# vbronetskyi/nclt-slam-project

Hardware: AMD Instinct MI355X
Metric: relocalization frames/sec @640x480, 10k-landmark DB; Hamming-match HBM GB/s (higher is better)
Workload: dtype u8; 1 GPU; 640x480 BGR frames, 10000-record landmark DB (640000 descriptors, rows=fixed64), global relocalization tick per frame: ORB(500) + whole-DB mutual Hamming scan + top-25 PnP-RANSAC(200); frames resident in HBM, every frame's 96-byte result record written to pinned host memory by the tick's last kernel; distinct_frames=32, preroll_steps=20, streams=4, records=10000, descriptors=640000, parallelism=frames sharded across ranks, database replicated, no collective

## Files before the change

nclt-slam-project_amd/csrc/reloc_ctx.hip:

```cpp
#include <stdarg.h>
#include <stdlib.h>

#include "reloc_internal.h"

static thread_local char g_err[512] = "";

void reloc_set_error(const char *fmt, ...)
{
    va_list ap;
    va_start(ap, fmt);
    vsnprintf(g_err, sizeof(g_err), fmt, ap);
    va_end(ap);
}

RELOC_API const char *reloc_last_error(void) { return g_err; }

RELOC_API int reloc_device_count(void)
{
    int n = 0;
    if (hipGetDeviceCount(&n) != hipSuccess) return 0;
    return n;
}

template <typename T>
static int dalloc(T **p, int64_t count)
{
    HIP_TRY(hipMalloc((void **)p, (size_t)(count > 0 ? count : 1) * sizeof(T)));
    return 0;
}

static int ctx_alloc(reloc_ctx *c)
{
    int rc = 0;
    const int64_t mf = c->max_feat;
    int64_t pyr = 0;
    for (int l = 0; l < NLEV; ++l) {
        double s = pow(RELOC_ORB_SCALE_FACTOR, (double)l);
        int64_t w = (int64_t)(c->max_w / s) + 2, h = (int64_t)(c->max_h / s) + 2;
        pyr += ((w + 63) / 64 * 64) * h + 256;
    }
    c->pyr_bytes = pyr;
    rc |= dalloc(&c->pyr, pyr);
    rc |= dalloc(&c->blur, pyr);
    rc |= dalloc(&c->nms, pyr);
    rc |= dalloc(&c->rz_tab, (int64_t)NLEV * 2 * 2 * (c->max_w > c->max_h ? c->max_w : c->max_h));
    rc |= dalloc((char **)&c->pyr_tiles, (int64_t)((c->max_w + 15) / 16) * ((c->max_h + 15) / 16) * 128);
    rc |= dalloc(&c->hist, NLEV * 256);
    rc |= dalloc(&c->cand_cnt, NLEV);
    rc |= dalloc(&c->cand_key, (int64_t)NLEV * RELOC_ORB_STAGE1_CAP);
    rc |= dalloc(&c->cand_resp, (int64_t)NLEV * RELOC_ORB_STAGE1_CAP);
    rc |= dalloc(&c->kp_cnt, NLEV);
    rc |= dalloc(&c->kp_key, (int64_t)NLEV * RELOC_ORB_STAGE1_CAP);
    rc |= dalloc(&c->kp_resp, (int64_t)NLEV * RELOC_ORB_STAGE1_CAP);
    rc |= dalloc(&c->f_xy, mf * 2);
    rc |= dalloc(&c->f_size, mf);
    rc |= dalloc(&c->f_angle, mf);
    rc |= dalloc(&c->f_resp, mf);
    rc |= dalloc(&c->f_oct, mf);
    rc |= dalloc(&c->f_desc, mf * 32);
    rc |= dalloc(&c->f_count, 1);
    rc |= dalloc(&c->frame_img, (int64_t)c->max_w * c->max_h * 3);
    rc |= dalloc((char **)&c->orb_const, 1024);
    rc |= dalloc(&c->dbg_cut, NLEV);
    rc |= dalloc(&c->cand_ids, MAX_CAND);
    rc |= dalloc(&c->cand_n, 1);
    rc |= dalloc(&c->m_qidx, (int64_t)MAX_CAND * MAX_REC_ROWS);
    rc |= dalloc(&c->m_tidx, (int64_t)MAX_CAND * MAX_REC_ROWS);
    rc |= dalloc(&c->m_dist, (int64_t)MAX_CAND * MAX_REC_ROWS);
    rc |= dalloc(&c->m_n, MAX_CAND);
    rc |= dalloc(&c->p_obj, (int64_t)MAX_CAND * MAX_REC_ROWS * 3);
    rc |= dalloc(&c->p_img, (int64_t)MAX_CAND * MAX_REC_ROWS * 2);
    rc |= dalloc(&c->p_Rt, (int64_t)MAX_CAND * MAX_HYP * 12);
    rc |= dalloc(&c->p_cnt, (int64_t)MAX_CAND * MAX_HYP);
    rc |= dalloc(&c->p_inl, (int64_t)MAX_CAND * MAX_REC_ROWS);
    rc |= dalloc(&c->p_out, MAX_CAND);
    rc |= dalloc(&c->tick_res, 1);
    if (hipHostMalloc((void **)&c->tick_res_host, sizeof(TickResult), hipHostMallocDefault) != hipSuccess) {
        reloc_set_error("hipHostMalloc(result record) failed");
        c->tick_res_host = nullptr;
// ... 301 lines not shown
```

nclt-slam-project_amd/csrc/reloc_internal.h:

```cpp
#pragma once
#include <hip/hip_runtime.h>
#include <stdint.h>
#include <stdio.h>
#include <string.h>

#include "../../include/reloc.h"
#include "../../include/reloc_spec.h"

#define RELOC_API extern "C" __attribute__((visibility("default")))
#define RELOC_PROF_RING 256

void reloc_set_error(const char *fmt, ...);

#define HIP_TRY(expr)                                                                      \
    do {                                                                                   \
        hipError_t e_ = (expr);                                                            \
        if (e_ != hipSuccess) {                                                            \
            reloc_set_error("%s failed: %s (%s:%d)", #expr, hipGetErrorString(e_), __FILE__, \
                            __LINE__);                                                     \
            return RELOC_E_HIP;                                                            \
        }                                                                                  \
    } while (0)

#define ARG_CHECK(cond, msg)                                 \
// ... 9 lines not shown
        if (!(c) || !(cond)) {                                \
            reloc_set_error("bad argument: %s", msg);         \
            return RELOC_E_ARG;                               \
        }                                                     \
        (void)hipSetDevice((c)->device);                      \
    } while (0)

constexpr int NLEV = RELOC_ORB_NLEVELS;
constexpr int MAX_REC_ROWS = 4096;
constexpr int MAX_CAND = 32;
constexpr int MAX_HYP = 1024;
constexpr int64_t MAX_DB_RECORDS = 0xFFFFF;

#ifndef RELOC_SCAN_NUM_VGPR
#define RELOC_SCAN_NUM_VGPR 104
#endif
#if RELOC_SCAN_NUM_VGPR > 0
#define RELOC_SCAN_VGPR_ATTR __attribute__((amdgpu_num_vgpr(RELOC_SCAN_NUM_VGPR / 2)))
#else
#define RELOC_SCAN_VGPR_ATTR
#endif
#ifndef RELOC_SMALL_PRIO
#define RELOC_SMALL_PRIO 3
#endif
#define RELOC_SMALL_KERNEL_PRIO() __builtin_amdgcn_s_setprio(RELOC_SMALL_PRIO)

struct OrbLevel {
    int w, h;
    int stride;
    int64_t off;
    float scale;
    int quota;
};

struct TickResult {
    double anchor_pose[7];
    double reproj;
    int32_t n_inl;
    int32_t lm_idx;
    int32_t outcome;
    int32_t n_candidates;
    int32_t n_features;
    int32_t relocating;
    int32_t pad[2];
};
static_assert(sizeof(TickResult) == 96, "TickResult is the 96-byte record documented in include/reloc.h");

struct AccumResult {
    double nearest_m;
    int32_t appended;
    int32_t n_kpts;
};

struct DbShare { int refs = 1; };

struct DbArena {
    DbShare *share = nullptr;
    int64_t cap_records = 0, cap_rows = 0;
    int64_t records = 0, rows = 0;
    int max_rows = 0;
    uint8_t *desc = nullptr;
    float *pts3d = nullptr;
    float *kp2d = nullptr;
    int64_t *off = nullptr;
    double *pose = nullptr;
    double *xy_heading = nullptr;
// ... 253 lines not shown
```

nclt-slam-project_amd/csrc/reloc_match.hip:

```cpp
#include <stdlib.h>
#include <new>
#include <type_traits>
#include <utility>

#include "reloc_internal.h"

typedef uint32_t u32;

__device__ __forceinline__ u32 bcnt_acc(u32 x, u32 acc)
{
    u32 r;
    asm("v_bcnt_u32_b32 %0, %1, %2" : "=v"(r) : "v"(x), "v"(acc));
    return r;
}
__device__ __forceinline__ u32 min_u16(u32 a, u32 b)
{
    u32 r;
    asm("v_min_u16 %0, %1, %2" : "=v"(r) : "v"(a), "v"(b));
    return r;
}
template <u32 IDX>
__device__ __forceinline__ u32 key_fma(u32 d, u32 c128)
{
    u32 r;
// ... 643 lines not shown
            }
#pragma unroll
    for (int j = 0; j < 4; ++j) hs[j] = add_lshl6(acc[j][0], acc[j][1]);
}

__device__ __forceinline__ void sq_load4(const uint4 *__restrict__ cur, int q0, int C, u32 (&qw)[4][8])
{
    const char *base = (const char *)cur;
#pragma unroll
    for (int jj = 0; jj < 4; ++jj) {
        const u32 o = (u32)min(q0 + jj, C - 1) << 5;
        const uint4 qa = *(const uint4 *)(base + o), qb = *(const uint4 *)(base + o + 16);
        qw[jj][0] = qa.x; qw[jj][1] = qa.y; qw[jj][2] = qa.z; qw[jj][3] = qa.w;
        qw[jj][4] = qb.x; qw[jj][5] = qb.y; qw[jj][6] = qb.z; qw[jj][7] = qb.w;
    }
}

#define SQ_N4(a, b)  "v_min_u16_dpp " a ", " a ", " a " row_shl:4 row_mask:0xf bank_mask:0x5\n\t" \
                     "v_min_u16_dpp " a ", " b ", " b " row_shr:4 row_mask:0xf bank_mask:0xa\n\t"
#define SQ_N8(a, b)  "v_min_u16_dpp " a ", " a ", " a " row_ror:8 row_mask:0xf bank_mask:0x3\n\t" \
                     "v_min_u16_dpp " a ", " b ", " b " row_ror:8 row_mask:0xf bank_mask:0xc\n\t"
#define SQ_Q1(a)     "v_min_u16_dpp " a ", " a ", " a " quad_perm:[1,0,3,2] row_mask:0xf bank_mask:0xf\n\t"
#define SQ_Q2(a)     "v_min_u16_dpp " a ", " a ", " a " quad_perm:[2,3,0,1] row_mask:0xf bank_mask:0xf\n\t"
#define SQ_NOP       "s_nop 1\n\t"
template <int G>
__device__ __forceinline__ u32 sq_bfly(u32 (&d)[G])
{
    if constexpr (G == 16) {
        asm volatile(SQ_NOP
                     SQ_N4("%0", "%1") SQ_N4("%2", "%3") SQ_N4("%4", "%5") SQ_N4("%6", "%7")
                     SQ_N4("%8", "%9") SQ_N4("%10", "%11") SQ_N4("%12", "%13") SQ_N4("%14", "%15")
                     SQ_N8("%0", "%2") SQ_N8("%4", "%6") SQ_N8("%8", "%10") SQ_N8("%12", "%14")
                     "v_permlane16_swap_b32 %0, %4\n\t"
                     "v_permlane16_swap_b32 %8, %12\n\t"
                     "v_min_u16 %0, %0, %4\n\t"
                     "v_min_u16 %8, %8, %12\n\t"
                     SQ_NOP
                     "v_permlane32_swap_b32 %0, %8\n\t"
                     "v_min_u16 %0, %0, %8\n\t"
                     SQ_NOP SQ_Q1("%0") SQ_NOP SQ_Q2("%0")
                     : "+v"(d[0]), "+v"(d[1]), "+v"(d[2]), "+v"(d[3]), "+v"(d[4]), "+v"(d[5]), "+v"(d[6]), "+v"(d[7]), "+v"(d[8]),
                       "+v"(d[9]), "+v"(d[10]), "+v"(d[11]), "+v"(d[12]), "+v"(d[13]), "+v"(d[14]), "+v"(d[15]));
    } else if constexpr (G == 8) {
        asm volatile(SQ_NOP
                     SQ_N4("%0", "%1") SQ_N4("%2", "%3") SQ_N4("%4", "%5") SQ_N4("%6", "%7")
                     SQ_N8("%0", "%2") SQ_N8("%4", "%6")
                     SQ_NOP
                     "v_permlane16_swap_b32 %0, %4\n\t"
                     "v_min_u16 %0, %0, %4\n\t"
                     SQ_NOP SQ_Q1("%0") SQ_NOP SQ_Q2("%0")
                     "v_mov_b32 %4, %0\n\t"
                     SQ_NOP
                     "v_permlane32_swap_b32 %0, %4\n\t"
                     "v_min_u16 %0, %0, %4\n\t"
                     : "+v"(d[0]), "+v"(d[1]), "+v"(d[2]), "+v"(d[3]), "+v"(d[4]), "+v"(d[5]), "+v"(d[6]), "+v"(d[7]));
    } else {
        static_assert(G == 4, "groups of 4, 8 or 16 queries");
        asm volatile(SQ_NOP
                     SQ_N4("%0", "%1") SQ_N4("%2", "%3")
                     SQ_NOP
                     SQ_N8("%0", "%2")
                     SQ_NOP SQ_Q1("%0") SQ_NOP SQ_Q2("%0")
                     "v_mov_b32 %2, %0\n\t"
                     SQ_NOP
                     "v_permlane16_swap_b32 %0, %2\n\t"
                     "v_min_u16 %0, %0, %2\n\t"
// ... 884 lines not shown
```

nclt-slam-project_amd/csrc/reloc_orb.hip:

```cpp
#include <math.h>

#include "../../include/reloc_orb_pattern.h"
#include "reloc_internal.h"

typedef uint32_t u32;

constexpr int HARRIS_CHUNK = 1024;
static_assert(HARRIS_CHUNK == 1024, "k_harris reads one dword per thread");

struct OrbTable {
    OrbLevel lev[NLEV];
    int fast_tile_base[NLEV + 1];
    int blur_tile_base[NLEV + 1];
    int flat_base[NLEV + 1];
    int rz_off[NLEV][4];
};

__constant__ signed char c_pattern[RELOC_ORB_NTESTS * 4];
__constant__ int c_umax[16] = {15, 15, 15, 15, 14, 14, 14, 13, 13, 12, 11, 10, 9, 8, 6, 3};
__constant__ signed char c_ring_dx[16] = {0, 1, 2, 3, 3, 3, 2, 1, 0, -1, -2, -3, -3, -3, -2, -1};
__constant__ signed char c_ring_dy[16] = {3, 3, 2, 1, 0, -1, -2, -3, -3, -3, -2, -1, 0, 1, 2, 3};

__device__ __forceinline__ int find_level(const int *base, int id)
{
// ... 13 lines not shown
    return p;
}

__device__ __forceinline__ int gray_fixed(int b, int g, int r, int flags)
{
    const bool c15 = flags & RELOC_GRAY_FLAG_15BIT;
    const int cb = c15 ? RELOC_GRAY15_CB : RELOC_GRAY_CB, cg = c15 ? RELOC_GRAY15_CG : RELOC_GRAY_CG, cr = c15 ? RELOC_GRAY15_CR : RELOC_GRAY_CR;
    const int sh = c15 ? RELOC_GRAY15_SHIFT : RELOC_GRAY_SHIFT;
    return (b * cb + g * cg + r * cr + (1 << (sh - 1))) >> sh;
}
static inline int gray_flags(const reloc_ctx *ctx, int order)
{
    return (order & 1) | (ctx->prm.gray_coeff_bits == RELOC_GRAY15_SHIFT ? RELOC_GRAY_FLAG_15BIT : 0);
}
__global__ __launch_bounds__(256) void k_gray_plain(const uint8_t *__restrict__ src, int w, int h, int sstride, int order_rgb,
                                                    uint8_t *__restrict__ dst)
{
    const int x = blockIdx.x * 256 + threadIdx.x, y = blockIdx.y;
    if (x >= w) return;
    const uint8_t *s = src + (size_t)y * sstride + 3 * x;
    const int c0 = s[0], c1 = s[1], c2 = s[2];
    const int b = (order_rgb & 1) ? c2 : c0, r = (order_rgb & 1) ? c0 : c2;
    dst[(size_t)y * w + x] = (uint8_t)gray_fixed(b, c1, r, order_rgb);
}

#ifndef PYR_TW
#define PYR_TW 64
#define PYR_TH 32
#endif
constexpr int PT_W = PYR_TW, PT_H = PYR_TH;
struct PyrTile {
    uint16_t o[NLEV][4];
    uint16_t n[NLEV][4];
};
static_assert(sizeof(PyrTile) == 128, "PyrTile is read as 8 dwordx4");

struct PyrLds { int lev[NLEV]; int tabs; };

struct OrbFrame {
    const OrbTable *tab; const PyrTile *tiles; const int32_t *rz; const uint8_t *src;
    uint8_t *pyr, *nms, *blur; int32_t *hist, *cand_cnt; u32 *cand_key; float *cand_resp; int32_t *dbg_cut;
    int32_t *kp_cnt; u32 *kp_key; float *kp_resp; float *f_xy, *f_size, *f_angle, *f_resp; int32_t *f_oct; uint8_t *f_desc;
    int32_t *f_count;
};
struct OrbBatch { OrbFrame f[RELOC_BATCH_MAX]; };

template <int CH, bool ALIGNED>
__device__ __forceinline__ void pyr_fetch(const uint8_t *sp, int x4, int w, u32 (&d)[3])
{
    if (ALIGNED) {
        const u32 *s4 = reinterpret_cast<const u32 *>(sp);
        d[0] = s4[0];
        if (CH == 3) { d[1] = s4[1]; d[2] = s4[2]; }
    } else {
        d[0] = d[1] = d[2] = 0;
#pragma unroll
        for (int k = 0; k < 4 * CH; ++k)
            if (x4 + k / CH < w) d[k >> 2] |= (u32)sp[k] << (8 * (k & 3));
    }
}

template <int CH>
__device__ __forceinline__ u32 pyr_gray4(const u32 (&d)[3], int x4, int w, int order_rgb)
{
    if (CH == 1) return d[0];
    u32 out = 0;
#pragma unroll
    for (int k = 0; k < 4; ++k) {
        int c[3];
#pragma unroll
        for (int j = 0; j < 3; ++j) { const int bi = 3 * k + j; c[j] = (d[bi >> 2] >> (8 * (bi & 3))) & 0xFF; }
        const int b = (order_rgb & 1) ? c[2] : c[0], r = (order_rgb & 1) ? c[0] : c[2];
        const int g = gray_fixed(b, c[1], r, order_rgb);
        if (x4 + k < w) out |= (u32)g << (8 * k);
    }
    return out;
}

__device__ __forceinline__ void pyr_tab_index(const OrbTable *__restrict__ tab, const PyrTile &T, const int (&tbase)[NLEV + 1], int i,
                                              int &po, int &pc)
{
    int j = i, nw = 0, x0 = 0, y0 = 0, ox = 0, cx = 0, oy = 0, cy = 0;
#pragma unroll
    for (int k = 1; k < NLEV; ++k) {
        const bool m = i >= tbase[k];
        j = m ? i - tbase[k] : j;
        nw = m ? T.n[k][1] - T.n[k][0] : nw;
        x0 = m ? (int)T.n[k][0] : x0;
        y0 = m ? (int)T.n[k][2] : y0;
        ox = m ? tab->rz_off[k][0] : ox;
        cx = m ? tab->rz_off[k][1] : cx;
        oy = m ? tab->rz_off[k][2] : oy;
        cy = m ? tab->rz_off[k][3] : cy;
    }
    const bool isx = j < nw;
    const int p = isx ? x0 + j : y0 + j - nw;
    po = (isx ? ox : oy) + p;
    pc = (isx ? cx : cy) + p;
}

__device__ __forceinline__ int pyr_div(int q, float inv) { return (int)(((float)q + 0.5f) * inv); }

template <int CH, bool ALIGNED, int PYR_BS>
__device__ __forceinline__ void pyramid_body(const OrbTable *__restrict__ tab, const PyrTile *__restrict__ tiles,
                                                 const int32_t *__restrict__ rz, const uint8_t *__restrict__ src, int w, int h,
                                                 int sstride, int order_rgb, uint8_t *__restrict__ pyr, PyrLds lds,
                                                 int32_t *__restrict__ hist, int32_t *__restrict__ cand_cnt)
{
    extern __shared__ u32 s_pyr[];
    const int tid = threadIdx.x;
    if (blockIdx.x == 0) {
        for (int i = tid; i < NLEV * 256; i += PYR_BS) hist[i] = 0;
        if (tid < NLEV) cand_cnt[tid] = 0;
    }
    const PyrTile &T = tiles[blockIdx.x];
    uint8_t *const base = reinterpret_cast<uint8_t *>(s_pyr);
    u32 *const tabs = s_pyr + (lds.tabs >> 2);
    int tbase[NLEV + 1];
    tbase[1] = 0;
#pragma unroll
    for (int l = 1; l < NLEV; ++l) tbase[l + 1] = tbase[l] + (T.n[l][1] - T.n[l][0]) + (T.n[l][3] - T.n[l][2]);
    constexpr int TAB_IT = 1024 / PYR_BS, L0_IT = 1536 / PYR_BS;
    u32 tv[TAB_IT][2];
#pragma unroll
    for (int it = 0; it < TAB_IT; ++it) {
        const int i = tid + it * PYR_BS;
        tv[it][0] = tv[it][1] = 0;
        if (i < tbase[NLEV]) {
            int po, pc;
            pyr_tab_index(tab, T, tbase, i, po, pc);
            tv[it][0] = (u32)rz[po];
            tv[it][1] = (u32)rz[pc];
        }
    }
    const int x00 = T.n[0][0], y00 = T.n[0][2], qpr0 = (T.n[0][1] - x00 + 3) >> 2, nq0 = qpr0 * (T.n[0][3] - y00);
    const float inv0 = 1.0f / (float)(qpr0 > 0 ? qpr0 : 1);
    u32 fv[L0_IT][3];
#pragma unroll
    for (int it = 0; it < L0_IT; ++it) {
        const int q = tid + it * PYR_BS;
        if (q < nq0) {
            const int ry = pyr_div(q, inv0), x4 = x00 + (q - ry * qpr0) * 4;
            pyr_fetch<CH, ALIGNED>(src + (size_t)(y00 + ry) * sstride + CH * x4, x4, w, fv[it]);
        }
    }
#pragma unroll
    for (int it = 0; it < TAB_IT; ++it) {
        const int i = tid + it * PYR_BS;
        if (i < tbase[NLEV]) tabs[i] = tv[it][0] | tv[it][1] << 16;
    }
#pragma unroll
    for (int it = 0; it < L0_IT; ++it) {
        const int q = tid + it * PYR_BS;
        if (q < nq0) {
            const int ry = pyr_div(q, inv0), x4 = x00 + (q - ry * qpr0) * 4;
            reinterpret_cast<u32 *>(base + lds.lev[0])[q] = pyr_gray4<CH>(fv[it], x4, w, order_rgb);
        }
    }
    for (int q = tid + L0_IT * PYR_BS; q < nq0; q += PYR_BS) {
        const int ry = pyr_div(q, inv0), x4 = x00 + (q - ry * qpr0) * 4;
        u32 d[3];
        pyr_fetch<CH, ALIGNED>(src + (size_t)(y00 + ry) * sstride + CH * x4, x4, w, d);
        reinterpret_cast<u32 *>(base + lds.lev[0])[q] = pyr_gray4<CH>(d, x4, w, order_rgb);
    }
    for (int i = tid + TAB_IT * PYR_BS; i < tbase[NLEV]; i += PYR_BS) {
        int po, pc;
        pyr_tab_index(tab, T, tbase, i, po, pc);
        tabs[i] = (u32)rz[po] | (u32)rz[pc] << 16;
    }
    __syncthreads();
#pragma unroll
    for (int l = 0; l + 1 < NLEV; ++l) {
        const int sw = tab->lev[l].w, sh = tab->lev[l].h;
        const uint8_t *cur = base + lds.lev[l];
        u32 *nxt = reinterpret_cast<u32 *>(base + lds.lev[l + 1]);
        const int nx0 = T.n[l][0], ny0 = T.n[l][2], pitch = ((T.n[l][1] - nx0 + 3) >> 2) << 2;
        const int dx0 = T.n[l + 1][0], dx1 = T.n[l + 1][1], dh = T.n[l + 1][3] - T.n[l + 1][2];
        const int qpr = (dx1 - dx0 + 3) >> 2;
        const u32 *xt = tabs + tbase[l + 1], *yt = xt + (dx1 - dx0);
        const u32 one = 1u << RELOC_RESIZE_COEF_BITS;
        const float inv = 1.0f / (float)(qpr > 0 ? qpr : 1);
        for (int q = tid; q < qpr * dh; q += PYR_BS) {
            const int ry = pyr_div(q, inv), rx4 = (q - ry * qpr) * 4;
            const u32 ye = yt[ry];
            const int sy0 = (int)(ye & 0xFFFF), sy1 = sy0 + 1 < sh ? sy0 + 1 : sh - 1;
            const u32 b = ye >> 16;
            const uint8_t *r0 = cur + (sy0 - ny0) * pitch - nx0, *r1 = cur + (sy1 - ny0) * pitch - nx0;
            u32 out = 0;
#pragma unroll
            for (int k = 0; k < 4; ++k) {
                if (dx0 + rx4 + k < dx1) {
                    const u32 xe = xt[rx4 + k];
                    const int k0 = (int)(xe & 0xFFFF), k1 = k0 + 1 < sw ? k0 + 1 : sw - 1;
                    const u32 a = xe >> 16;
                    const u32 h0 = (u32)r0[k0] * (one - a) + (u32)r0[k1] * a;
                    const u32 h1 = (u32)r1[k0] * (one - a) + (u32)r1[k1] * a;
                    const u32 v = h0 * (one - b) + h1 * b;
                    out |= ((v + (1u << 15)) >> 16) << (8 * k);
                }
            }
            nxt[q] = out;
        }
        __syncthreads();
    }
#pragma unroll
    for (int l = 0; l < NLEV; ++l) {
        const OrbLevel L = tab->lev[l];
        const uint8_t *cur = base + lds.lev[l];
        const int nx0 = T.n[l][0], ny0 = T.n[l][2], pitch = ((T.n[l][1] - nx0 + 3) >> 2) << 2;
        const int x0 = T.o[l][0], x1 = T.o[l][1], y0 = T.o[l][2], oh = T.o[l][3] - y0;
        const int qpr = (x1 - x0) >> 2;
        uint8_t *dst = pyr + L.off;
        const float inv = 1.0f / (float)(qpr > 0 ? qpr : 1);
        for (int q = tid; q < qpr * oh; q += PYR_BS) {
            const int ry = pyr_div(q, inv), x4 = x0 + (q - ry * qpr) * 4;
            u32 v = 0;
            if (x4 < L.w) {
                v = *reinterpret_cast<const u32 *>(cur + (y0 + ry - ny0) * pitch + (x4 - nx0));
                if (x4 + 4 > L.w) v &= 0xFFFFFFFFu >> (8 * (x4 + 4 - L.w));
            }
            *reinterpret_cast<u32 *>(dst + (size_t)(y0 + ry) * L.stride + x4) = v;
        }
    }
}
template <int CH, bool ALIGNED, int PYR_BS>
__global__ __launch_bounds__(PYR_BS) void k_pyramid(const OrbTable *__restrict__ tab, const PyrTile *__restrict__ tiles,
                                                 const int32_t *__restrict__ rz, const uint8_t *__restrict__ src, int w, int h,
                                                 int sstride, int order_rgb, uint8_t *__restrict__ pyr, PyrLds lds,
                                                 int32_t *__restrict__ hist, int32_t *__restrict__ cand_cnt)
{
    RELOC_SMALL_KERNEL_PRIO();
    pyramid_body<CH, ALIGNED, PYR_BS>(tab, tiles, rz, src, w, h, sstride, order_rgb, pyr, lds, hist, cand_cnt);
}
template <int CH, bool ALIGNED, int PYR_BS>
__global__ __launch_bounds__(PYR_BS) void k_pyramid_batch(OrbBatch b, int w, int h, int sstride, int order_rgb, PyrLds lds)
{
    RELOC_SMALL_KERNEL_PRIO();
    const OrbFrame &F = b.f[blockIdx.y];
    pyramid_body<CH, ALIGNED, PYR_BS>(F.tab, F.tiles, F.rz, F.src, w, h, sstride, order_rgb, F.pyr, lds, F.hist, F.cand_cnt);
}


template <bool REFLECT>
__device__ __forceinline__ u32 halo_dword(const uint8_t *__restrict__ row, int gx, int w)
{
    if (gx >= 0 && gx + 4 <= w) return *reinterpret_cast<const u32 *>(row + gx);
    u32 v = 0;
#pragma unroll
    for (int k = 0; k < 4; ++k) {
        const int x = REFLECT ? reflect101(gx + k, w) : min(max(gx + k, 0), w - 1);
        v |= (u32)row[x] << (8 * k);
    }
    return v;
}
// ... 726 lines not shown
    OrbTable tab;
    memset(&tab, 0, sizeof(tab));
    int64_t off = 0;
    for (int l = 0; l < NLEV; ++l) {
        const float s = (float)pow(RELOC_ORB_SCALE_FACTOR, (double)l);
        OrbLevel &L = tab.lev[l];
        L.scale = s;
        L.w = (int)lrintf((float)w / s);
        L.h = (int)lrintf((float)h / s);
        L.stride = (L.w + 63) / 64 * 64;
        L.off = off;
        off += ((int64_t)L.stride * L.h + 255) / 256 * 256;
    }
    if (off > ctx->pyr_bytes) { reloc_set_error("pyramid arena too small"); return RELOC_E_CAPACITY; }
    {
        const float factor = (float)(1.0 / RELOC_ORB_SCALE_FACTOR);
        float nper = (float)(nfeatures * (1 - factor) / (1 - (float)pow((double)factor, (double)NLEV)));
        int sum = 0;
        for (int l = 0; l < NLEV - 1; ++l) {
            tab.lev[l].quota = (int)lrintf(nper);
            sum += tab.lev[l].quota;
            nper *= factor;
        }
        tab.lev[NLEV - 1].quota = nfeatures - sum > 0 ? nfeatures - sum : 0;
    }
    for (int l = 0; l < NLEV; ++l) {
        const OrbLevel &L = tab.lev[l];
        tab.fast_tile_base[l + 1] = tab.fast_tile_base[l] + (L.stride / FT) * ((L.h + FT - 1) / FT);
        tab.blur_tile_base[l + 1] = tab.blur_tile_base[l] + ((L.w + BT_W - 1) / BT_W) * ((L.h + BT_H - 1) / BT_H);
        tab.flat_base[l + 1] = tab.flat_base[l] + (int)(((int64_t)L.stride * L.h + HARRIS_CHUNK - 1) / HARRIS_CHUNK);
    }
    const int maxdim = ctx->max_w > ctx->max_h ? ctx->max_w : ctx->max_h;
    int32_t *host = (int32_t *)malloc(sizeof(int32_t) * (size_t)NLEV * 4 * maxdim);
    int pos = 0;
    for (int l = 1; l < NLEV; ++l) {
        const OrbLevel &S = tab.lev[l - 1], &D = tab.lev[l];
        tab.rz_off[l][0] = pos; tab.rz_off[l][1] = pos + D.w;
        resize_axis(S.w, D.w, host + pos, host + pos + D.w);
        pos += 2 * D.w;
        tab.rz_off[l][2] = pos; tab.rz_off[l][3] = pos + D.h;
        resize_axis(S.h, D.h, host + pos, host + pos + D.h);
        pos += 2 * D.h;
    }
    const int ntx = (w + PT_W - 1) / PT_W, nty = (h + PT_H - 1) / PT_H;
    PyrTile *tiles = (PyrTile *)calloc((size_t)ntx * nty, sizeof(PyrTile));
    int lds_lev[NLEV] = {}, lds_t = 0;
    for (int t = 0; t < ntx * nty; ++t) {
        const int tx = t % ntx, ty = t / ntx;
        PyrTile &T = tiles[t];
        int nx0 = 0, nx1 = 0, ny0 = 0, ny1 = 0;
        int tsum = 0;
        for (int l = NLEV - 1; l >= 0; --l) {
            const OrbLevel &L = tab.lev[l];
            const int quads = (l == 0 ? (L.w + 3) / 4 : L.stride / 4);
            const int ox0 = 4 * (int)((int64_t)tx * quads / ntx), ox1 = 4 * (int)((int64_t)(tx + 1) * quads / ntx);
            const int oy0 = (int)((int64_t)ty * L.h / nty), oy1 = (int)((int64_t)(ty + 1) * L.h / nty);
            T.o[l][0] = (uint16_t)ox0; T.o[l][1] = (uint16_t)ox1; T.o[l][2] = (uint16_t)oy0; T.o[l][3] = (uint16_t)oy1;
            int cx0 = ox0, cx1 = ox1 < L.w ? ox1 : L.w, cy0 = oy0, cy1 = oy1;
            const bool stores = ox0 < ox1 && oy0 < oy1;
            const bool own = cx0 < cx1 && cy0 < cy1, need = nx0 < nx1 && ny0 < ny1;
            if (need) {
                const int32_t *xo = host + tab.rz_off[l + 1][0], *yo = host + tab.rz_off[l + 1][2];
                int sx0 = xo[nx0], sx1 = xo[nx1 - 1] + 2, sy0 = yo[ny0], sy1 = yo[ny1 - 1] + 2;
                if (sx1 > L.w) sx1 = L.w;
                if (sy1 > L.h) sy1 = L.h;
                if (own) {
                    cx0 = cx0 < sx0 ? cx0 : sx0; cx1 = cx1 > sx1 ? cx1 : sx1;
                    cy0 = cy0 < sy0 ? cy0 : sy0; cy1 = cy1 > sy1 ? cy1 : sy1;
                } else {
                    cx0 = sx0; cx1 = sx1; cy0 = sy0; cy1 = sy1;
                }
            } else if (!own) {
                cx0 = cx1 = cy0 = cy1 = 0;
            }
            cx0 &= ~3;
            T.n[l][0] = (uint16_t)cx0; T.n[l][1] = (uint16_t)cx1; T.n[l][2] = (uint16_t)cy0; T.n[l][3] = (uint16_t)cy1;
            if (!stores) T.o[l][0] = T.o[l][1] = T.o[l][2] = T.o[l][3] = 0;
            nx0 = cx0; nx1 = cx1; ny0 = cy0; ny1 = cy1;
            const int bytes = ((cx1 - cx0 + 3) / 4 * 4) * (cy1 - cy0);
            lds_lev[l] = bytes > lds_lev[l] ? bytes : lds_lev[l];
            if (l >= 1) tsum += (cx1 - cx0) + (cy1 - cy0);
        }
        lds_t = tsum > lds_t ? tsum : lds_t;
    }
    ctx->pyr_ntiles = ntx * nty;
    {
        int o = 0;
        for (int l = 0; l < NLEV; ++l) { ctx->pyr_lds[l] = o; o += (lds_lev[l] + 15) / 16 * 16; }
        ctx->pyr_lds[NLEV] = o;
        ctx->pyr_lds_bytes = o + 4 * lds_t;
    }
    if (ctx->pyr_lds_bytes > 64 * 1024) { free(host); free(tiles); reloc_set_error("pyramid tile exceeds LDS"); return RELOC_E_CAPACITY; }
    hipError_t e0 = hipMemcpyAsync(ctx->pyr_tiles, tiles, sizeof(PyrTile) * (size_t)ntx * nty, hipMemcpyHostToDevice, ctx->stream);
    hipError_t e1 = hipMemcpyAsync(ctx->rz_tab, host, sizeof(int32_t) * (size_t)pos, hipMemcpyHostToDevice, ctx->stream);
    hipError_t e2 = hipMemcpyAsync(ctx->orb_const, &tab, sizeof(tab), hipMemcpyHostToDevice, ctx->stream);
    hipError_t e3 = hipStreamSynchronize(ctx->stream);
    free(host);
    free(tiles);
    HIP_TRY(e0); HIP_TRY(e1); HIP_TRY(e2); HIP_TRY(e3);
    memcpy(ctx->lev, tab.lev, sizeof(tab.lev));
    memcpy(ctx->orb_tab_host, &tab, sizeof(tab));
    ctx->orb_w = w; ctx->orb_h = h; ctx->orb_nfeat = nfeatures;
    return RELOC_OK;
}

struct ClaheGeom {
    int w, h;
    int tx, ty;
    int tw, th;
    int clip;
    float lut_scale;
    float inv_tw, inv_th;
};
struct ClaheFrames { const uint8_t *src[RELOC_BATCH_MAX]; uint8_t *lut[RELOC_BATCH_MAX]; uint8_t *dst[RELOC_BATCH_MAX]; };
#ifndef RELOC_CLAHE_LUT_BS
#define RELOC_CLAHE_LUT_BS 1024
#endif
constexpr int CLAHE_LUT_BS = RELOC_CLAHE_LUT_BS;
constexpr int CLAHE_MAX_TILES = RELOC_CLAHE_MAX_TILES;

static ClaheGeom clahe_geom(int w, int h, double clip_limit, int tx, int ty)
{
    ClaheGeom g;
    g.w = w; g.h = h; g.tx = tx; g.ty = ty;
    const bool divides = w % tx == 0 && h % ty == 0;
    g.tw = divides ? w / tx : (w + tx - w % tx) / tx;
    g.th = divides ? h / ty : (h + ty - h % ty) / ty;
    const int area = g.tw * g.th;
    if (clip_limit > 0.0) {
        const int c = (int)(clip_limit * area / 256);
// ... 61 lines not shown
            hb[k] += batch + (residual && bin % step == 0 && bin / step < residual ? 1 : 0);
        }
    }
    int loc[4];
    loc[0] = hb[0];
#pragma unroll
    for (int k = 1; k < 4; ++k) loc[k] = loc[k - 1] + hb[k];
    int incl = loc[3];
#pragma unroll
    for (int off = 1; off < 64; off <<= 1) {
        const int t = __shfl_up(incl, off);
        if (lane >= off) incl += t;
    }
    const int excl = incl - loc[3];
    u32 out = 0;
#pragma unroll
    for (int k = 0; k < 4; ++k) {
        int v = __float2int_rn((float)(excl + loc[k]) * g.lut_scale);
        v = v < 0 ? 0 : (v > 255 ? 255 : v);
        out |= (u32)v << (8 * k);
    }
    reinterpret_cast<u32 *>(F.lut[blockIdx.y] + (size_t)blockIdx.x * 256)[lane] = out;
}

template <int CH, bool ALIGNED>
__global__ __launch_bounds__(256) void k_clahe_apply(ClaheFrames F, ClaheGeom g, int sstride, int flags, int dstride)
{
    const int quads = (g.w + 3) >> 2;
    const int q = blockIdx.x * 256 + threadIdx.x;
    if (q >= quads * g.h) return;
    const int y = q / quads, x4 = 4 * (q - y * quads);
    u32 d[3];
    pyr_fetch<CH, ALIGNED>(F.src[blockIdx.y] + (size_t)y * sstride + CH * x4, x4, g.w, d);
    const u32 gray4 = pyr_gray4<CH>(d, x4, g.w, flags);
    const float tyf = (float)y * g.inv_th - 0.5f;
    int ty1 = (int)floorf(tyf);
    const float ya = tyf - (float)ty1, ya1 = 1.0f - ya;
    const int ty2 = ty1 + 1 < g.ty - 1 ? ty1 + 1 : g.ty - 1;
    ty1 = ty1 > 0 ? ty1 : 0;
    const uint8_t *lut = F.lut[blockIdx.y];
    const uint8_t *L1 = lut + (size_t)ty1 * g.tx * 256, *L2 = lut + (size_t)ty2 * g.tx * 256;
    u32 out = 0;
#pragma unroll
    for (int k = 0; k < 4; ++k) {
        const int x = x4 + k;
        const float txf = (float)x * g.inv_tw - 0.5f;
        int tx1 = (int)floorf(txf);
        const float xa = txf - (float)tx1, xa1 = 1.0f - xa;
        const int tx2 = tx1 + 1 < g.tx - 1 ? tx1 + 1 : g.tx - 1;
        tx1 = tx1 > 0 ? tx1 : 0;
        const int v = (gray4 >> (8 * k)) & 0xFF;
        const float l11 = L1[tx1 * 256 + v], l12 = L1[tx2 * 256 + v], l21 = L2[tx1 * 256 + v], l22 = L2[tx2 * 256 + v];
        const float res = (l11 * xa1 + l12 * xa) * ya1 + (l21 * xa1 + l22 * xa) * ya;
        int r = __float2int_rn(res);
        r = r < 0 ? 0 : (r > 255 ? 255 : r);
        if (x < g.w) out |= (u32)r << (8 * k);
    }
    uint8_t *dst = F.dst[blockIdx.y] + (size_t)y * dstride + x4;
    if ((dstride & 3) == 0) {
        *reinterpret_cast<u32 *>(dst) = out;
    } else {
#pragma unroll
        for (int k = 0; k < 4; ++k)
            if (x4 + k < g.w) dst[k] = (uint8_t)(out >> (8 * k));
    }
}

// ... 513 lines not shown
```

Measured before the change: 7444 frames/s.

## Rewrite pyramid build with packed resize records, udot4 gray/bilinear and mul-shift row indexing

The ORB pyramid kernel now precomputes per-quad resize records on the host: byte-select masks, packed 8-bit weights and column offsets. The device then bilinearly downsamples four pixels at a time with alignbyte, perm and udot4 instead of per-pixel scalar math. BGR-to-gray conversion also uses udot4, row/column splitting uses a precomputed 20-bit reciprocal multiply instead of float division, and tile and table metadata are read through constant address space. The change cuts ALU work and LDS table lookups in the pyramid stage, in exchange for larger tile records, added host-side table building, weight precision narrowed to 8 bits, and a geometry check that can reject some level sizes. It also adds an s_nop between the permlane swaps in the match reduction.

```diff
diff --git a/nclt-slam-project_amd/csrc/reloc_ctx.hip b/nclt-slam-project_amd/csrc/reloc_ctx.hip
--- a/nclt-slam-project_amd/csrc/reloc_ctx.hip
+++ b/nclt-slam-project_amd/csrc/reloc_ctx.hip
@@ -43,8 +43,8 @@
     rc |= dalloc(&c->pyr, pyr);
     rc |= dalloc(&c->blur, pyr);
     rc |= dalloc(&c->nms, pyr);
-    rc |= dalloc(&c->rz_tab, (int64_t)NLEV * 2 * 2 * (c->max_w > c->max_h ? c->max_w : c->max_h));
-    rc |= dalloc((char **)&c->pyr_tiles, (int64_t)((c->max_w + 15) / 16) * ((c->max_h + 15) / 16) * 128);
+    rc |= dalloc(&c->rz_tab, (int64_t)orb_rz_words(c->max_w, c->max_h));
+    rc |= dalloc((char **)&c->pyr_tiles, (int64_t)((c->max_w + 15) / 16) * ((c->max_h + 15) / 16) * 256);
     rc |= dalloc(&c->hist, NLEV * 256);
     rc |= dalloc(&c->cand_cnt, NLEV);
     rc |= dalloc(&c->cand_key, (int64_t)NLEV * RELOC_ORB_STAGE1_CAP);
diff --git a/nclt-slam-project_amd/csrc/reloc_internal.h b/nclt-slam-project_amd/csrc/reloc_internal.h
--- a/nclt-slam-project_amd/csrc/reloc_internal.h
+++ b/nclt-slam-project_amd/csrc/reloc_internal.h
@@ -65,6 +65,8 @@
     float scale;
     int quota;
 };
+
+static inline size_t orb_rz_words(int max_w, int max_h) { return (size_t)(NLEV - 1) * (3 * ((size_t)max_w + 3) + (size_t)max_h + 8); }
 
 struct TickResult {
     double anchor_pose[7];
diff --git a/nclt-slam-project_amd/csrc/reloc_match.hip b/nclt-slam-project_amd/csrc/reloc_match.hip
--- a/nclt-slam-project_amd/csrc/reloc_match.hip
+++ b/nclt-slam-project_amd/csrc/reloc_match.hip
@@ -699,6 +699,7 @@
                      SQ_N4("%8", "%9") SQ_N4("%10", "%11") SQ_N4("%12", "%13") SQ_N4("%14", "%15")
                      SQ_N8("%0", "%2") SQ_N8("%4", "%6") SQ_N8("%8", "%10") SQ_N8("%12", "%14")
                      "v_permlane16_swap_b32 %0, %4\n\t"
+                     "s_nop 0\n\t"
                      "v_permlane16_swap_b32 %8, %12\n\t"
                      "v_min_u16 %0, %0, %4\n\t"
                      "v_min_u16 %8, %8, %12\n\t"
diff --git a/nclt-slam-project_amd/csrc/reloc_orb.hip b/nclt-slam-project_amd/csrc/reloc_orb.hip
--- a/nclt-slam-project_amd/csrc/reloc_orb.hip
+++ b/nclt-slam-project_amd/csrc/reloc_orb.hip
@@ -69,8 +69,12 @@
 struct PyrTile {
     uint16_t o[NLEV][4];
     uint16_t n[NLEV][4];
+    uint32_t mn[NLEV];
+    uint32_t mo[NLEV];
 };
-static_assert(sizeof(PyrTile) == 128, "PyrTile is read as 8 dwordx4");
+static_assert(sizeof(PyrTile) == 192, "PyrTile is read by scalar loads; reloc_ctx.hip sizes ctx->pyr_tiles by it");
+#define PYR_CONST(T) T __attribute__((address_space(4)))
+constexpr int PYR_REC = 12;
 
 struct PyrLds { int lev[NLEV]; int tabs; };
 
@@ -98,45 +102,35 @@
 }
 
 template <int CH>
-__device__ __forceinline__ u32 pyr_gray4(const u32 (&d)[3], int x4, int w, int order_rgb)
+__device__ __forceinline__ u32 pyr_gray4(const u32 (&d)[3], int order_rgb)
 {
     if (CH == 1) return d[0];
-    u32 out = 0;
-#pragma unroll
-    for (int k = 0; k < 4; ++k) {
-        int c[3];
-#pragma unroll
-        for (int j = 0; j < 3; ++j) { const int bi = 3 * k + j; c[j] = (d[bi >> 2] >> (8 * (bi & 3))) & 0xFF; }
-        const int b = (order_rgb & 1) ? c[2] : c[0], r = (order_rgb & 1) ? c[0] : c[2];
-        const int g = gray_fixed(b, c[1], r, order_rgb);
-        if (x4 + k < w) out |= (u32)g << (8 * k);
-    }
-    return out;
-}
-
-__device__ __forceinline__ void pyr_tab_index(const OrbTable *__restrict__ tab, const PyrTile &T, const int (&tbase)[NLEV + 1], int i,
-                                              int &po, int &pc)
-{
-    int j = i, nw = 0, x0 = 0, y0 = 0, ox = 0, cx = 0, oy = 0, cy = 0;
-#pragma unroll
-    for (int k = 1; k < NLEV; ++k) {
-        const bool m = i >= tbase[k];
-        j = m ? i - tbase[k] : j;
-        nw = m ? T.n[k][1] - T.n[k][0] : nw;
-        x0 = m ? (int)T.n[k][0] : x0;
-        y0 = m ? (int)T.n[k][2] : y0;
-        ox = m ? tab->rz_off[k][0] : ox;
-        cx = m ? tab->rz_off[k][1] : cx;
-        oy = m ? tab->rz_off[k][2] : oy;
-        cy = m ? tab->rz_off[k][3] : cy;
-    }
-    const bool isx = j < nw;
-    const int p = isx ? x0 + j : y0 + j - nw;
-    po = (isx ? ox : oy) + p;
-    pc = (isx ? cx : cy) + p;
-}
-
-__device__ __forceinline__ int pyr_div(int q, float inv) { return (int)(((float)q + 0.5f) * inv); }
+    const bool c15 = order_rgb & RELOC_GRAY_FLAG_15BIT;
+    const u32 cb = c15 ? (u32)RELOC_GRAY15_CB << (16 - RELOC_GRAY15_SHIFT) : (u32)RELOC_GRAY_CB << (16 - RELOC_GRAY_SHIFT);
+    const u32 cg = c15 ? (u32)RELOC_GRAY15_CG << (16 - RELOC_GRAY15_SHIFT) : (u32)RELOC_GRAY_CG << (16 - RELOC_GRAY_SHIFT);
+    const u32 cr = c15 ? (u32)RELOC_GRAY15_CR << (16 - RELOC_GRAY15_SHIFT) : (u32)RELOC_GRAY_CR << (16 - RELOC_GRAY_SHIFT);
+    const u32 c0 = (order_rgb & 1) ? cr : cb, c2 = (order_rgb & 1) ? cb : cr;
+    const u32 wl = (c0 & 0xFF) | (cg & 0xFF) << 8 | (c2 & 0xFF) << 16, wh = (c0 >> 8) | (cg >> 8) << 8 | (c2 >> 8) << 16;
+    u32 p[4], g[4];
+    p[0] = d[0];
+    p[1] = __builtin_amdgcn_alignbyte(d[1], d[0], 3);
+    p[2] = __builtin_amdgcn_alignbyte(d[2], d[1], 2);
+    p[3] = d[2] >> 8;
+#pragma unroll
+    for (int k = 0; k < 4; ++k)
+        g[k] = (__builtin_amdgcn_udot4(p[k], wh, 0u, false) << 8) + __builtin_amdgcn_udot4(p[k], wl, 1u << 15, false);
+    return __builtin_amdgcn_perm(g[1], g[0], 0x0c0c0602u) | __builtin_amdgcn_perm(g[3], g[2], 0x06020c0cu);
+}
+
+__device__ __forceinline__ int pyr_row(int q, u32 m) { return (int)(__umul24((u32)q, m) >> 20); }
+
+__device__ __forceinline__ int pyr_pick(const int (&base)[NLEV + 1], const int (&v)[NLEV], int i)
+{
+    int r = v[1];
+#pragma unroll
+    for (int k = 2; k < NLEV; ++k) r += i >= base[k] ? v[k] - v[k - 1] : 0;
+    return r;
+}
 
 template <int CH, bool ALIGNED, int PYR_BS>
 __device__ __forceinline__ void pyramid_body(const OrbTable *__restrict__ tab, const PyrTile *__restrict__ tiles,
@@ -146,117 +140,118 @@
 {
     extern __shared__ u32 s_pyr[];
     const int tid = threadIdx.x;
+    const PYR_CONST(PyrTile) &T = *(const PYR_CONST(PyrTile) *)(tiles + blockIdx.x);
+    const PYR_CONST(OrbTable) &G = *(const PYR_CONST(OrbTable) *)tab;
     if (blockIdx.x == 0) {
         for (int i = tid; i < NLEV * 256; i += PYR_BS) hist[i] = 0;
         if (tid < NLEV) cand_cnt[tid] = 0;
     }
-    const PyrTile &T = tiles[blockIdx.x];
     uint8_t *const base = reinterpret_cast<uint8_t *>(s_pyr);
-    u32 *const tabs = s_pyr + (lds.tabs >> 2);
-    int tbase[NLEV + 1];
-    tbase[1] = 0;
-#pragma unroll
-    for (int l = 1; l < NLEV; ++l) tbase[l + 1] = tbase[l] + (T.n[l][1] - T.n[l][0]) + (T.n[l][3] - T.n[l][2]);
-    constexpr int TAB_IT = 1024 / PYR_BS, L0_IT = 1536 / PYR_BS;
-    u32 tv[TAB_IT][2];
-#pragma unroll
-    for (int it = 0; it < TAB_IT; ++it) {
-        const int i = tid + it * PYR_BS;
-        tv[it][0] = tv[it][1] = 0;
-        if (i < tbase[NLEV]) {
-            int po, pc;
-            pyr_tab_index(tab, T, tbase, i, po, pc);
-            tv[it][0] = (u32)rz[po];
-            tv[it][1] = (u32)rz[pc];
-        }
-    }
-    const int x00 = T.n[0][0], y00 = T.n[0][2], qpr0 = (T.n[0][1] - x00 + 3) >> 2, nq0 = qpr0 * (T.n[0][3] - y00);
-    const float inv0 = 1.0f / (float)(qpr0 > 0 ? qpr0 : 1);
+    uint4 *const recs = reinterpret_cast<uint4 *>(s_pyr + (lds.tabs >> 2));
+    int nq[NLEV], nh[NLEV], rb[NLEV + 1], yb[NLEV + 1], rdelta[NLEV], ydelta[NLEV];
+#pragma unroll
+    for (int l = 0; l < NLEV; ++l) { nq[l] = (T.n[l][1] - T.n[l][0] + 3) >> 2; nh[l] = T.n[l][3] - T.n[l][2]; }
+    rb[0] = rb[1] = yb[0] = yb[1] = 0;
+    rdelta[0] = ydelta[0] = 0;
+#pragma unroll
+    for (int l = 1; l < NLEV; ++l) {
+        rb[l + 1] = rb[l] + 3 * nq[l];
+        yb[l + 1] = yb[l] + nh[l];
+        rdelta[l] = (G.rz_off[l][0] >> 2) + 3 * (T.n[l][0] >> 2) - rb[l];
+        ydelta[l] = G.rz_off[l][2] + T.n[l][2] - yb[l];
+    }
+    u32 *const ytab = reinterpret_cast<u32 *>(recs + rb[NLEV]);
+    const uint4 *rz4 = reinterpret_cast<const uint4 *>(rz);
+    uint4 rv = make_uint4(0, 0, 0, 0);
+    u32 yv = 0;
+    if (tid < rb[NLEV]) rv = rz4[tid + pyr_pick(rb, rdelta, tid)];
+    if (tid < yb[NLEV]) yv = (u32)rz[tid + pyr_pick(yb, ydelta, tid)];
+    constexpr int L0_IT = 1536 / PYR_BS;
+    const int x00 = T.n[0][0], y00 = T.n[0][2], qpr0 = nq[0], nq0 = qpr0 * nh[0];
+    const u32 m0 = T.mn[0];
     u32 fv[L0_IT][3];
 #pragma unroll
     for (int it = 0; it < L0_IT; ++it) {
         const int q = tid + it * PYR_BS;
         if (q < nq0) {
-            const int ry = pyr_div(q, inv0), x4 = x00 + (q - ry * qpr0) * 4;
+            const int ry = pyr_row(q, m0), x4 = x00 + (q - ry * qpr0) * 4;
             pyr_fetch<CH, ALIGNED>(src + (size_t)(y00 + ry) * sstride + CH * x4, x4, w, fv[it]);
         }
     }
-#pragma unroll
-    for (int it = 0; it < TAB_IT; ++it) {
-        const int i = tid + it * PYR_BS;
-        if (i < tbase[NLEV]) tabs[i] = tv[it][0] | tv[it][1] << 16;
-    }
+    if (tid < rb[NLEV]) recs[tid] = rv;
+    if (tid < yb[NLEV]) ytab[tid] = yv;
 #pragma unroll
     for (int it = 0; it < L0_IT; ++it) {
         const int q = tid + it * PYR_BS;
-        if (q < nq0) {
-            const int ry = pyr_div(q, inv0), x4 = x00 + (q - ry * qpr0) * 4;
-            reinterpret_cast<u32 *>(base + lds.lev[0])[q] = pyr_gray4<CH>(fv[it], x4, w, order_rgb);
-        }
+        if (q < nq0) reinterpret_cast<u32 *>(base + lds.lev[0])[q] = pyr_gray4<CH>(fv[it], order_rgb);
     }
     for (int q = tid + L0_IT * PYR_BS; q < nq0; q += PYR_BS) {
-        const int ry = pyr_div(q, inv0), x4 = x00 + (q - ry * qpr0) * 4;
+        const int ry = pyr_row(q, m0), x4 = x00 + (q - ry * qpr0) * 4;
         u32 d[3];
         pyr_fetch<CH, ALIGNED>(src + (size_t)(y00 + ry) * sstride + CH * x4, x4, w, d);
-        reinterpret_cast<u32 *>(base + lds.lev[0])[q] = pyr_gray4<CH>(d, x4, w, order_rgb);
-    }
-    for (int i = tid + TAB_IT * PYR_BS; i < tbase[NLEV]; i += PYR_BS) {
-        int po, pc;
-        pyr_tab_index(tab, T, tbase, i, po, pc);
-        tabs[i] = (u32)rz[po] | (u32)rz[pc] << 16;
-    }
+        reinterpret_cast<u32 *>(base + lds.lev[0])[q] = pyr_gray4<CH>(d, order_rgb);
+    }
+    for (int i = tid + PYR_BS; i < rb[NLEV]; i += PYR_BS) recs[i] = rz4[i + pyr_pick(rb, rdelta, i)];
+    for (int i = tid + PYR_BS; i < yb[NLEV]; i += PYR_BS) ytab[i] = (u32)rz[i + pyr_pick(yb, ydelta, i)];
     __syncthreads();
 #pragma unroll
     for (int l = 0; l + 1 < NLEV; ++l) {
-        const int sw = tab->lev[l].w, sh = tab->lev[l].h;
-        const uint8_t *cur = base + lds.lev[l];
         u32 *nxt = reinterpret_cast<u32 *>(base + lds.lev[l + 1]);
-        const int nx0 = T.n[l][0], ny0 = T.n[l][2], pitch = ((T.n[l][1] - nx0 + 3) >> 2) << 2;
-        const int dx0 = T.n[l + 1][0], dx1 = T.n[l + 1][1], dh = T.n[l + 1][3] - T.n[l + 1][2];
-        const int qpr = (dx1 - dx0 + 3) >> 2;
-        const u32 *xt = tabs + tbase[l + 1], *yt = xt + (dx1 - dx0);
-        const u32 one = 1u << RELOC_RESIZE_COEF_BITS;
-        const float inv = 1.0f / (float)(qpr > 0 ? qpr : 1);
-        for (int q = tid; q < qpr * dh; q += PYR_BS) {
-            const int ry = pyr_div(q, inv), rx4 = (q - ry * qpr) * 4;
+        const int pitch = nq[l] << 2;
+        const int cbase = lds.lev[l] - T.n[l][2] * pitch - T.n[l][0];
+        const int qpr = nq[l + 1], nquad = qpr * nh[l + 1];
+        const u32 m = T.mn[l + 1];
+        const uint4 *rec = recs + rb[l + 1];
+        const u32 *yt = ytab + yb[l + 1];
+        for (int q = tid; q < nquad; q += PYR_BS) {
+            const int ry = pyr_row(q, m), rx = q - ry * qpr;
             const u32 ye = yt[ry];
-            const int sy0 = (int)(ye & 0xFFFF), sy1 = sy0 + 1 < sh ? sy0 + 1 : sh - 1;
-            const u32 b = ye >> 16;
-            const uint8_t *r0 = cur + (sy0 - ny0) * pitch - nx0, *r1 = cur + (sy1 - ny0) * pitch - nx0;
-            u32 out = 0;
+            const uint4 sel = rec[3 * rx], wgt = rec[3 * rx + 1];
+            const uint2 col = *reinterpret_cast<const uint2 *>(rec + 3 * rx + 2);
+            const u32 b = ye >> 16, nb = (1u << RELOC_RESIZE_COEF_BITS) - b;
+            const u32 *r0 = reinterpret_cast<const u32 *>(base + (cbase + (int)__umul24(ye & 0xFFFF, (u32)pitch) + (int)col.x));
+            const u32 *r1 = r0 + nq[l];
+            const u32 a0 = r0[0], a1 = r0[1], a2 = r0[2], b0 = r1[0], b1 = r1[1], b2 = r1[2];
+            const u32 lo0 = __builtin_amdgcn_alignbyte(a1, a0, col.y), hi0 = __builtin_amdgcn_alignbyte(a2, a1, col.y);
+            const u32 lo1 = __builtin_amdgcn_alignbyte(b1, b0, col.y), hi1 = __builtin_amdgcn_alignbyte(b2, b1, col.y);
+            const u32 s[4] = {sel.x, sel.y, sel.z, sel.w}, c[4] = {wgt.x, wgt.y, wgt.z, wgt.w};
+            u32 v[4];
 #pragma unroll
             for (int k = 0; k < 4; ++k) {
-                if (dx0 + rx4 + k < dx1) {
-                    const u32 xe = xt[rx4 + k];
-                    const int k0 = (int)(xe & 0xFFFF), k1 = k0 + 1 < sw ? k0 + 1 : sw - 1;
-                    const u32 a = xe >> 16;
-                    const u32 h0 = (u32)r0[k0] * (one - a) + (u32)r0[k1] * a;
-                    const u32 h1 = (u32)r1[k0] * (one - a) + (u32)r1[k1] * a;
-                    const u32 v = h0 * (one - b) + h1 * b;
-                    out |= ((v + (1u << 15)) >> 16) << (8 * k);
+                const u32 h0 = __builtin_amdgcn_udot4(__builtin_amdgcn_perm(hi0, lo0, s[k]), c[k], 0u, false);
+                const u32 h1 = __builtin_amdgcn_udot4(__builtin_amdgcn_perm(hi1, lo1, s[k]), c[k], 0u, false);
+                v[k] = __umul24(h0, nb) + (__umul24(h1, b) + (1u << 15));
+            }
+            nxt[q] = __builtin_amdgcn_perm(v[1], v[0], 0x0c0c0602u) | __builtin_amdgcn_perm(v[3], v[2], 0x06020c0cu);
+        }
+        __syncthreads();
+    }
+#pragma unroll
+    for (int l = 0; l < NLEV; ++l) {
+        const int lw = G.lev[l].w, lstride = G.lev[l].stride;
+        const int pitch = nq[l] << 2;
+        const int x0 = T.o[l][0], x1 = T.o[l][1], y0 = T.o[l][2], oh = T.o[l][3] - y0;
+        const int qpr = (x1 - x0) >> 2, nquad = qpr * oh;
+        const u32 m = T.mo[l];
+        const int cbase = lds.lev[l] + (y0 - T.n[l][2]) * pitch + (x0 - T.n[l][0]);
+        uint8_t *dst = pyr + G.lev[l].off + (size_t)y0 * lstride + x0;
+        if (x1 <= lw) {
+#pragma clang loop unroll(disable) vectorize(disable) interleave(disable)
+            for (int q = tid; q < nquad; q += PYR_BS) {
+                const int ry = pyr_row(q, m), rx4 = (q - ry * qpr) << 2;
+                *reinterpret_cast<u32 *>(dst + (u32)(ry * lstride + rx4)) = *reinterpret_cast<const u32 *>(base + (cbase + ry * pitch + rx4));
+            }
+        } else {
+#pragma clang loop unroll(disable) vectorize(disable) interleave(disable)
+            for (int q = tid; q < nquad; q += PYR_BS) {
+                const int ry = pyr_row(q, m), rx4 = (q - ry * qpr) << 2, left = lw - x0 - rx4;
+                u32 v = 0;
+                if (left > 0) {
+                    v = *reinterpret_cast<const u32 *>(base + (cbase + ry * pitch + rx4));
+                    if (left < 4) v &= 0xFFFFFFFFu >> (8 * (4 - left));
                 }
+                *reinterpret_cast<u32 *>(dst + (u32)(ry * lstride + rx4)) = v;
             }
-            nxt[q] = out;
-        }
-        __syncthreads();
-    }
-#pragma unroll
-    for (int l = 0; l < NLEV; ++l) {
-        const OrbLevel L = tab->lev[l];
-        const uint8_t *cur = base + lds.lev[l];
-        const int nx0 = T.n[l][0], ny0 = T.n[l][2], pitch = ((T.n[l][1] - nx0 + 3) >> 2) << 2;
-        const int x0 = T.o[l][0], x1 = T.o[l][1], y0 = T.o[l][2], oh = T.o[l][3] - y0;
-        const int qpr = (x1 - x0) >> 2;
-        uint8_t *dst = pyr + L.off;
-        const float inv = 1.0f / (float)(qpr > 0 ? qpr : 1);
-        for (int q = tid; q < qpr * oh; q += PYR_BS) {
-            const int ry = pyr_div(q, inv), x4 = x0 + (q - ry * qpr) * 4;
-            u32 v = 0;
-            if (x4 < L.w) {
-                v = *reinterpret_cast<const u32 *>(cur + (y0 + ry - ny0) * pitch + (x4 - nx0));
-                if (x4 + 4 > L.w) v &= 0xFFFFFFFFu >> (8 * (x4 + 4 - L.w));
-            }
-            *reinterpret_cast<u32 *>(dst + (size_t)(y0 + ry) * L.stride + x4) = v;
         }
     }
 }
@@ -1049,19 +1044,49 @@
     }
     const int maxdim = ctx->max_w > ctx->max_h ? ctx->max_w : ctx->max_h;
     int32_t *host = (int32_t *)malloc(sizeof(int32_t) * (size_t)NLEV * 4 * maxdim);
-    int pos = 0;
+    const size_t dev_cap = orb_rz_words(ctx->max_w, ctx->max_h);
+    int32_t *dev = (int32_t *)calloc(dev_cap, sizeof(int32_t));
+    int hoff[NLEV][4] = {};
+    int pos = 0, dpos = 0;
+    bool rec_ok = true;
     for (int l = 1; l < NLEV; ++l) {
         const OrbLevel &S = tab.lev[l - 1], &D = tab.lev[l];
-        tab.rz_off[l][0] = pos; tab.rz_off[l][1] = pos + D.w;
+        hoff[l][0] = pos; hoff[l][1] = pos + D.w;
         resize_axis(S.w, D.w, host + pos, host + pos + D.w);
         pos += 2 * D.w;
-        tab.rz_off[l][2] = pos; tab.rz_off[l][3] = pos + D.h;
+        hoff[l][2] = pos; hoff[l][3] = pos + D.h;
         resize_axis(S.h, D.h, host + pos, host + pos + D.h);
         pos += 2 * D.h;
-    }
+        const int32_t *xo = host + hoff[l][0], *xc = host + hoff[l][1], *yo = host + hoff[l][2], *yc = host + hoff[l][3];
+        const int nrec = (D.w + 3) / 4;
+        if ((size_t)dpos + (size_t)PYR_REC * nrec + D.h + 4 > dev_cap) { rec_ok = false; break; }
+        tab.rz_off[l][0] = tab.rz_off[l][1] = dpos;
+        for (int c = 0; c < nrec; ++c) {
+            uint32_t *r = (uint32_t *)dev + dpos + PYR_REC * c;
+            int first = 0;
+            for (int j = 0; j < 4; ++j) {
+                const int x = 4 * c + j;
+                if (x >= D.w) { r[j] = 0x0c0c0c0cu; r[4 + j] = 0; continue; }
+                int k0 = xo[x], a = xc[x];
+                if (a == (1 << RELOC_RESIZE_COEF_BITS)) { k0 += 1; a = 0; }
+                if (j == 0) first = k0;
+                const int rel = k0 - first;
+                if (rel < 0 || rel + 1 > 7 || a < 0 || a > 255) rec_ok = false;
+                r[j] = (uint32_t)rel | (uint32_t)(rel + 1) << 8 | (uint32_t)rel << 16 | 0x0cu << 24;
+                r[4 + j] = (uint32_t)(255 - a) | (uint32_t)a << 8 | 1u << 16;
+            }
+            r[8] = (uint32_t)(first & ~3);
+            r[9] = (uint32_t)(first & 3);
+        }
+        dpos += PYR_REC * nrec;
+        tab.rz_off[l][2] = tab.rz_off[l][3] = dpos;
+        for (int y = 0; y < D.h; ++y) dev[dpos + y] = (int32_t)((uint32_t)yo[y] | (uint32_t)yc[y] << 16);
+        dpos = (dpos + D.h + 3) & ~3;
+    }
+    if (!rec_ok) { free(host); free(dev); reloc_set_error("pyramid resize tables: unsupported level geometry"); return RELOC_E_CAPACITY; }
     const int ntx = (w + PT_W - 1) / PT_W, nty = (h + PT_H - 1) / PT_H;
     PyrTile *tiles = (PyrTile *)calloc((size_t)ntx * nty, sizeof(PyrTile));
-    int lds_lev[NLEV] = {}, lds_t = 0;
+    int lds_lev[NLEV] = {}, lds_t = 0, lds_pitch = 0;
     for (int t = 0; t < ntx * nty; ++t) {
         const int tx = t % ntx, ty = t / ntx;
         PyrTile &T = tiles[t];
@@ -1077,7 +1102,7 @@
             const bool stores = ox0 < ox1 && oy0 < oy1;
             const bool own = cx0 < cx1 && cy0 < cy1, need = nx0 < nx1 && ny0 < ny1;
             if (need) {
-                const int32_t *xo = host + tab.rz_off[l + 1][0], *yo = host + tab.rz_off[l + 1][2];
+                const int32_t *xo = host + hoff[l + 1][0], *yo = host + hoff[l + 1][2];
                 int sx0 = xo[nx0], sx1 = xo[nx1 - 1] + 2, sy0 = yo[ny0], sy1 = yo[ny1 - 1] + 2;
                 if (sx1 > L.w) sx1 = L.w;
                 if (sy1 > L.h) sy1 = L.h;
@@ -1096,7 +1121,11 @@
             nx0 = cx0; nx1 = cx1; ny0 = cy0; ny1 = cy1;
             const int bytes = ((cx1 - cx0 + 3) / 4 * 4) * (cy1 - cy0);
             lds_lev[l] = bytes > lds_lev[l] ? bytes : lds_lev[l];
-            if (l >= 1) tsum += (cx1 - cx0) + (cy1 - cy0);
+            if (l >= 1) tsum += 4 * PYR_REC * ((cx1 - cx0 + 3) / 4) + 4 * (cy1 - cy0);
+            const int ow = T.o[l][1] - T.o[l][0], nw4 = (cx1 - cx0 + 3) / 4;
+            T.mn[l] = (1u << 20) / (uint32_t)(nw4 > 0 ? nw4 : 1) + 1;
+            T.mo[l] = (1u << 20) / (uint32_t)(ow > 0 ? ow / 4 : 1) + 1;
+            lds_pitch = 4 * nw4 > lds_pitch ? 4 * nw4 : lds_pitch;
         }
         lds_t = tsum > lds_t ? tsum : lds_t;
     }
@@ -1105,14 +1134,15 @@
         int o = 0;
         for (int l = 0; l < NLEV; ++l) { ctx->pyr_lds[l] = o; o += (lds_lev[l] + 15) / 16 * 16; }
         ctx->pyr_lds[NLEV] = o;
-        ctx->pyr_lds_bytes = o + 4 * lds_t;
-    }
-    if (ctx->pyr_lds_bytes > 64 * 1024) { free(host); free(tiles); reloc_set_error("pyramid tile exceeds LDS"); return RELOC_E_CAPACITY; }
+        ctx->pyr_lds_bytes = o + lds_t + lds_pitch + 16;
+    }
+    if (ctx->pyr_lds_bytes > 64 * 1024) { free(host); free(dev); free(tiles); reloc_set_error("pyramid tile exceeds LDS"); return RELOC_E_CAPACITY; }
     hipError_t e0 = hipMemcpyAsync(ctx->pyr_tiles, tiles, sizeof(PyrTile) * (size_t)ntx * nty, hipMemcpyHostToDevice, ctx->stream);
-    hipError_t e1 = hipMemcpyAsync(ctx->rz_tab, host, sizeof(int32_t) * (size_t)pos, hipMemcpyHostToDevice, ctx->stream);
+    hipError_t e1 = hipMemcpyAsync(ctx->rz_tab, dev, sizeof(int32_t) * (size_t)dpos, hipMemcpyHostToDevice, ctx->stream);
     hipError_t e2 = hipMemcpyAsync(ctx->orb_const, &tab, sizeof(tab), hipMemcpyHostToDevice, ctx->stream);
     hipError_t e3 = hipStreamSynchronize(ctx->stream);
     free(host);
+    free(dev);
     free(tiles);
     HIP_TRY(e0); HIP_TRY(e1); HIP_TRY(e2); HIP_TRY(e3);
     memcpy(ctx->lev, tab.lev, sizeof(tab.lev));
@@ -1240,7 +1270,7 @@
     const int y = q / quads, x4 = 4 * (q - y * quads);
     u32 d[3];
     pyr_fetch<CH, ALIGNED>(F.src[blockIdx.y] + (size_t)y * sstride + CH * x4, x4, g.w, d);
-    const u32 gray4 = pyr_gray4<CH>(d, x4, g.w, flags);
+    const u32 gray4 = pyr_gray4<CH>(d, flags);
     const float tyf = (float)y * g.inv_th - 0.5f;
     int ty1 = (int)floorf(tyf);
     const float ya = tyf - (float)ty1, ya1 = 1.0f - ya;
```

New measurement: 7500 frames/s (median of 6 runs). About the same (+0.8%).
